# zgcr/SimpleAICV_pytorch_training_examples

Hardware: AMD Instinct MI355X
Metric: training images/sec/node (higher is better)
Workload: dtype bf16; 1 GPU; resnet50 3x224x224 synthetic training step (fwd+loss+bwd+all-reduce+optimizer), per-GPU batch 256; model=resnet50, global_batch=256, per_gpu_batch=256, parallelism=dp1, step_graph=True, bn_statistics=fixed-order partial rows, deterministic=True, loop=tools.scripts.train_classification, optimizer=SGD, param_groups=2

## Files before the change

### simpleaicv_pytorch_training_examples_amd/csrc/capi.hip

```cpp
#include <stdarg.h>
#include <stdio.h>
#include <string.h>

#include "common.h"
#include "saicv_internal.h"
#include "../../include/saicv_hip.h"

namespace saicv {

static thread_local char g_err[512] = "";

void set_error(const char* fmt, ...) {
    va_list ap;
    va_start(ap, fmt);
    vsnprintf(g_err, sizeof(g_err), fmt, ap);
    va_end(ap);
}

int check_launch(const char* what) {
    const hipError_t e = hipGetLastError();
    if (e != hipSuccess) {
        set_error("%s: launch failed: %s", what, hipGetErrorString(e));
        return -2;
    }
// ... 98 lines not shown
    return pack_weight(dtype, w, sO, sI, sR, sS, O, I, R, Sx, Ip, Op, wf, wd, S(stream));
}
int saicv_unpack_wgrad(const float* dw, int O, int I, int R, int Sx, int Ip, float* grad, long sO,
                       long sI, long sR, long sS, int accumulate, void* stream) {
    return unpack_wgrad(dw, O, I, R, Sx, Ip, grad, sO, sI, sR, sS, accumulate, S(stream));
}

int saicv_pack_weight_batched(int dtype, const saicv_pack_desc* descs, int n, int total_tiles, void* stream) {
    return pack_weight_batched(dtype, descs, n, total_tiles, S(stream));
}
int saicv_pack_input_s2d(int dtype, const float* src, long sN, long sC, long sH, long sW, void* dst, int N, int C, int H,
                         int W, int pad, int Cq, void* stream) {
    return pack_input_s2d(dtype, src, sN, sC, sH, sW, dst, N, C, H, W, pad, Cq, S(stream));
}
int saicv_pack_weight_s2d(int dtype, const float* w, long sO, long sI, long sR, long sS, int O, int I, int R, int Sx,
                          int Cq, void* wf, void* stream) {
    return pack_weight_s2d(dtype, w, sO, sI, sR, sS, O, I, R, Sx, Cq, wf, S(stream));
}
int saicv_unpack_wgrad_s2d(const float* dw, int O, int I, int R, int Sx, int Cq, float* grad, long sO, long sI, long sR,
                           long sS, int accumulate, void* stream) {
    return unpack_wgrad_s2d(dw, O, I, R, Sx, Cq, grad, sO, sI, sR, sS, accumulate, S(stream));
}

int saicv_conv2d_stat_rows(const saicv_conv_desc* d) {
    if (!d) return -1;
    return conv_stat_rows(d);
}

int saicv_conv2d_fwd(const saicv_conv_desc* d, const void* x, const void* wf, const float* bias,
                     void* y, int out_f32, float* stat_sum, float* stat_sq, void* stream) {
    if (check_desc(d, "saicv_conv2d_fwd")) return -1;
    SAICV_REQUIRE(!(stat_sum && out_f32), "saicv_conv2d_fwd: BN statistics need out_f32 = 0");
    const int M = d->N * d->OH * d->OW;
    return igemm_nt(d->dtype, 0, x, wf, y, bias, stat_sum, stat_sq, d->H, d->W, d->C, d->OH, d->OW,
                    d->R, d->S, d->stride, d->pad, M, d->K, d->R * d->S * d->C, d->K, out_f32, S(stream));
}

int saicv_conv2d_dgrad(const saicv_conv_desc* d, const void* dy, const void* wd, void* dx,
                       void* stream) {
    if (check_desc(d, "saicv_conv2d_dgrad")) return -1;
    const int M = d->N * d->H * d->W;
    return igemm_nt(d->dtype, 1, dy, wd, dx, nullptr, nullptr, nullptr, d->OH, d->OW, d->K, d->H, d->W,
                    d->R, d->S, d->stride, d->pad, M, d->C, d->R * d->S * d->K, d->C, 0, S(stream));
}

int saicv_conv2d_wgrad(const saicv_conv_desc* d, const void* dy, const void* x, float* dw,
                       void* stream) {
    if (check_desc(d, "saicv_conv2d_wgrad")) return -1;
    const int M = d->N * d->OH * d->OW;
    return igemm_tn(d->dtype, dy, x, dw, d->H, d->W, d->C, d->OH, d->OW, d->R, d->S, d->stride, d->pad,
                    M, d->K, d->R * d->S * d->C, S(stream));
}

int saicv_conv2d_wgrad_bias(const saicv_conv_desc* d, const void* dy, const void* x, float* dw, float* dbias,
                            void* stream) {
    if (check_desc(d, "saicv_conv2d_wgrad_bias")) return -1;
    const int M = d->N * d->OH * d->OW;
    return igemm_tn(d->dtype, dy, x, dw, d->H, d->W, d->C, d->OH, d->OW, d->R, d->S, d->stride, d->pad,
                    M, d->K, d->R * d->S * d->C, S(stream), dbias);
}

int saicv_linear_fwd(int dtype, const void* x, const void* wf, const float* bias, void* y, int M, int K, int N,
                     int out_f32, const void* addend, const float* row_scale, int rows_per_scale, void* stream) {
    EpiExtra ex;
    ex.addend = addend; ex.row_scale = row_scale; ex.rows_per_scale = rows_per_scale > 0 ? rows_per_scale : 1;
    return igemm_nt(dtype, 0, x, wf, y, bias, nullptr, nullptr, 1, 1, K, 1, 1, 1, 1, 1, 0, M, N, K, N, out_f32,
                    S(stream), (addend || row_scale) ? &ex : nullptr);
}
int saicv_linear_dgrad(int dtype, const void* dy, const void* wd, void* dx, int M, int K, int N, const void* addend,
                       void* stream) {
    EpiExtra ex;
    ex.addend = addend;
    return igemm_nt(dtype, 1, dy, wd, dx, nullptr, nullptr, nullptr, 1, 1, N, 1, 1, 1, 1, 1, 0, M, K, N, K, 0,
                    S(stream), addend ? &ex : nullptr);
}
int saicv_linear_gelu_fwd(int dtype, const void* x, const void* wf, const float* bias, void* y_pre, void* y_act, int M,
                          int K, int N, void* stream) {
    EpiExtra ex;
    ex.act_mode = 1; ex.out2 = y_act;
    return igemm_nt(dtype, 0, x, wf, y_pre, bias, nullptr, nullptr, 1, 1, K, 1, 1, 1, 1, 1, 0, M, N, K, N, 0, S(stream), &ex);
}
int saicv_linear_dgrad_gelu(int dtype, const void* dy, const void* wd, const void* pre, void* dx, int M, int K, int N,
                            void* stream) {
    EpiExtra ex;
    ex.act_mode = 2; ex.addend = pre;
    return igemm_nt(dtype, 1, dy, wd, dx, nullptr, nullptr, nullptr, 1, 1, N, 1, 1, 1, 1, 1, 0, M, K, N, K, 0, S(stream), &ex);
}
int saicv_linear_gelu_fwd_aux(int dtype, const void* x, const void* wf, const float* bias, void* y_dact, void* y_act, int M,
                              int K, int N, void* stream) {
    EpiExtra ex;
    ex.act_mode = 3; ex.out2 = y_act;
    return igemm_nt(dtype, 0, x, wf, y_dact, bias, nullptr, nullptr, 1, 1, K, 1, 1, 1, 1, 1, 0, M, N, K, N, 0, S(stream), &ex);
}
int saicv_linear_dgrad_mul(int dtype, const void* dy, const void* wd, const void* factor, void* dx, int M, int K, int N,
                           void* stream) {
    EpiExtra ex;
    ex.act_mode = 4; ex.addend = factor;
    return igemm_nt(dtype, 1, dy, wd, dx, nullptr, nullptr, nullptr, 1, 1, N, 1, 1, 1, 1, 1, 0, M, K, N, K, 0, S(stream), &ex);
}
int saicv_linear_wgrad(int dtype, const void* dy, const void* x, float* dw, float* dbias, int M, int K, int N,
                       void* stream) {
    return igemm_tn(dtype, dy, x, dw, 1, 1, K, 1, 1, 1, 1, 1, 0, M, N, K, S(stream), dbias);
}
int saicv_conv2d_dgrad_add(const saicv_conv_desc* d, const void* dy, const void* wd, const void* addend, void* dx,
                           void* stream) {
    if (check_desc(d, "saicv_conv2d_dgrad_add")) return -1;
// ... 312 lines not shown
```

### simpleaicv_pytorch_training_examples_amd/csrc/det.h

```cpp
#pragma once
#include <hip/hip_runtime.h>
#include <stddef.h>

namespace saicv {

extern int g_deterministic;

struct DetSink {
    float* part;
    size_t n;
};

__device__ __forceinline__ void det_add(const DetSink& s, float* dst_elem, size_t part_idx, int part_id, float v) {
    if (s.part) s.part[(size_t)part_id * s.n + part_idx] = v;
    else unsafeAtomicAdd(dst_elem, v);
}

struct DetParts {
    DetSink s{nullptr, 0};
    int nparts = 0;
    hipStream_t st = nullptr;
    int begin(hipStream_t stream, int parts, size_t n, const char* who, bool zero = true);
    int fold(float* dst, size_t offset, size_t count, bool wide = false) const;
    bool on() const { return s.part != nullptr; }
    const DetSink& sink() const { return s; }
};

}
```

### simpleaicv_pytorch_training_examples_amd/csrc/det.hip

```cpp
#include <mutex>

#include "common.h"
#include "det.h"

namespace saicv {

int g_deterministic = 0;

namespace {

struct StreamWs { hipStream_t st; float* p; size_t floats; };
constexpr size_t kInitialFloats = (size_t)24 << 20;
constexpr int MAX_STREAMS = 8;
StreamWs g_ws[MAX_STREAMS] = {};
int g_nws = 0;
StreamWs g_capture = {nullptr, nullptr, 0};
size_t g_max_floats = 0;
std::mutex g_mu;

bool is_capturing(hipStream_t st) {
    hipStreamCaptureStatus cap = hipStreamCaptureStatusNone;
    if (hipStreamIsCapturing(st, &cap) != hipSuccess) { (void)hipGetLastError(); return false; }
    return cap != hipStreamCaptureStatusNone;
}
// ... 48 lines not shown
    if (i >= count) return;
    const float* p = part + off + i;
    float acc = p[0];
    for (int k = 1; k < nparts; ++k) acc += p[(size_t)k * n];
    dst[i] += acc;
}
__global__ __launch_bounds__(256) void det_fold4_kernel(const float* __restrict__ part, size_t n, int nparts, size_t off, size_t count4,
                                                        float* __restrict__ dst) {
    const size_t i = (size_t)blockIdx.x * 256 + threadIdx.x;
    if (i >= count4) return;
    const float* p = part + off + i * 4;
    f32x4 acc = *reinterpret_cast<const f32x4*>(p);
    for (int k = 1; k < nparts; ++k) acc += *reinterpret_cast<const f32x4*>(p + (size_t)k * n);
    f32x4* d = reinterpret_cast<f32x4*>(dst + i * 4);
    *d = *d + acc;
}
constexpr int COOP_J = 8, COOP_E = 256 / COOP_J, COOP_CH = 32;
__global__ __launch_bounds__(256) void det_fold4_coop_kernel(const float* __restrict__ part, size_t n, int nparts, size_t off, size_t count4,
                                                             float* __restrict__ dst) {
    __shared__ f32x4 buf[2][COOP_CH][COOP_E];
    const int e = threadIdx.x % COOP_E, j = threadIdx.x / COOP_E;
    const size_t i = (size_t)blockIdx.x * COOP_E + e;
    const bool live = i < count4;
    const float* p = part + off + (live ? i : 0) * 4;
    const int chunks = (nparts + COOP_CH - 1) / COOP_CH;
    auto load = [&](int c) {
        f32x4 v[COOP_CH / COOP_J];
#pragma unroll
        for (int t = 0; t < COOP_CH / COOP_J; ++t) {
            const int k = c * COOP_CH + t * COOP_J + j;
            v[t] = (live && k < nparts) ? *reinterpret_cast<const f32x4*>(p + (size_t)k * n) : f32x4{0.f, 0.f, 0.f, 0.f};
        }
#pragma unroll
        for (int t = 0; t < COOP_CH / COOP_J; ++t) buf[c & 1][t * COOP_J + j][e] = v[t];
    };
    f32x4 acc = {0.f, 0.f, 0.f, 0.f};
    load(0);
    __syncthreads();
    for (int c = 0; c < chunks; ++c) {
        if (c + 1 < chunks) load(c + 1);
        if (j == 0) {
            const int cnt = min(COOP_CH, nparts - c * COOP_CH);
            int kk = 0;
            if (c == 0) { acc = buf[0][0][e]; kk = 1; }
            for (; kk < cnt; ++kk) acc += buf[c & 1][kk][e];
        }
        __syncthreads();
    }
    if (j == 0 && live) {
        f32x4* d = reinterpret_cast<f32x4*>(dst + i * 4);
        *d = *d + acc;
    }
}
constexpr int FOLD_J = 8, FOLD_E = 256 / FOLD_J;
__global__ __launch_bounds__(256) void det_fold4_wide_kernel(const float* __restrict__ part, size_t n, int nparts, size_t off, size_t count4,
                                                             float* __restrict__ dst) {
    __shared__ f32x4 red[FOLD_J][FOLD_E];
    const int e = threadIdx.x % FOLD_E, j = threadIdx.x / FOLD_E;
    const size_t i = (size_t)blockIdx.x * FOLD_E + e;
    f32x4 acc = {0.f, 0.f, 0.f, 0.f};
    if (i < count4) {
        const float* p = part + off + i * 4;
#pragma unroll 4
        for (int k = j; k < nparts; k += FOLD_J) acc += *reinterpret_cast<const f32x4*>(p + (size_t)k * n);
    }
    red[j][e] = acc;
    __syncthreads();
    if (j == 0 && i < count4) {
        f32x4 a = red[0][e];
#pragma unroll
        for (int jj = 1; jj < FOLD_J; ++jj) a += red[jj][e];
        f32x4* d = reinterpret_cast<f32x4*>(dst + i * 4);
        *d = *d + a;
    }
}

}

int DetParts::begin(hipStream_t stream, int parts, size_t n, const char* who, bool zero) {
    s = DetSink{nullptr, n};
    nparts = parts;
    st = stream;
    if (!g_deterministic || parts <= 1 || n == 0) return 0;
    float* p = ws_for(stream, (size_t)parts * n, who);
    if (!p) return -1;
    static const bool force = getenv("SAICV_ORDERED_ZERO") && atoi(getenv("SAICV_ORDERED_ZERO")) != 0;
    const bool clear = zero || force;
    if (clear && hipMemsetAsync(p, 0, (size_t)parts * n * sizeof(float), stream) != hipSuccess) {
        set_error("%s: clearing the deterministic workspace failed: %s", who, hipGetErrorString(hipGetLastError()));
        return -1;
    }
    s.part = p;
    return 0;
}

int DetParts::fold(float* dst, size_t offset, size_t count, bool wide_ok) const {
    if (!s.part || count == 0) return 0;
    const bool vec = (s.n % 4 == 0) && (offset % 4 == 0) && (count % 4 == 0) && ((uintptr_t)dst % 16 == 0);
    if (vec && wide_ok && nparts >= 4 * FOLD_J)
        hipLaunchKernelGGL(det_fold4_wide_kernel, dim3((unsigned)((count / 4 + FOLD_E - 1) / FOLD_E)), dim3(256), 0, st, s.part, s.n, nparts, offset, count / 4, dst);
    else if (vec && nparts >= COOP_CH)
        hipLaunchKernelGGL(det_fold4_coop_kernel, dim3((unsigned)((count / 4 + COOP_E - 1) / COOP_E)), dim3(256), 0, st, s.part, s.n, nparts, offset, count / 4, dst);
    else if (vec)
        hipLaunchKernelGGL(det_fold4_kernel, dim3((unsigned)((count / 4 + 255) / 256)), dim3(256), 0, st, s.part, s.n, nparts, offset, count / 4, dst);
    else
        hipLaunchKernelGGL(det_fold_kernel, dim3((unsigned)((count + 255) / 256)), dim3(256), 0, st, s.part, s.n, nparts, offset, count, dst);
    return check_launch("det_fold");
}

}

extern "C" {

int saicv_set_deterministic(int on) {
    const int prev = saicv::g_deterministic;
    saicv::g_deterministic = on ? 1 : 0;
    return prev;
}

int saicv_get_deterministic(void) { return saicv::g_deterministic; }

int saicv_deterministic_prepare(void* stream) {
    return saicv::ws_for((hipStream_t)stream, saicv::kInitialFloats, "deterministic_prepare") ? 0 : -1;
}

}
```

### simpleaicv_pytorch_training_examples_amd/csrc/igemm.hip

```cpp
#include <type_traits>

#include <stdlib.h>
#include "common.h"
#include "saicv_internal.h"
#include "det.h"
#include "../../include/saicv_hip.h"

namespace {

struct FastDiv {
    uint32_t mul, s1, s2;
};
DEVINL uint32_t fdiv(uint32_t n, FastDiv d) {
    const uint32_t t = __umulhi(d.mul, n);
    return (t + ((n - t) >> d.s1)) >> d.s2;
}

constexpr int nt_stages(int bm, int bn) { return (bm == 256 && bn == 128) ? 3 : 4; }
constexpr int nt_stages_kc8(int bm, int bn) { return (bm + bn) * 128 * 3 <= 150 * 1024 ? 3 : 2; }

struct NTParams {
    const void* src;
    const void* wgt;
    void* out;
// ... 753 lines not shown
        }
        __syncthreads();
        const size_t prow = (size_t)((MODE == 1 && cs > 1) ? blockIdx.y : 0) * p.bs_rows + tile_m;
        for (int c = tid; c < 2 * BN_T; c += NTHREADS) {
            const int which = c / BN_T, col = c - which * BN_T;
            float a = 0.f;
            for (int r = 0; r < RPP; ++r) a += red[(r * 2 + which) * BN_T + col];
            const int n = tile_n * BN_T + col;
            if (n < p.Nn) {
                float* dst = (which ? p.bs_gx : p.bs_g) + (p.stat_atomic_rows ? prow % p.stat_atomic_rows : prow) * (size_t)p.Nn + n;
                if (p.stat_atomic_rows) unsafeAtomicAdd(dst, a); else *dst = a;
            }
        }
    }
    }
#ifdef SAICV_NT_TIMELINE
    if (tl_on && tix == (int)blockIdx.x) {
        NT_STAMP(6);
        asm volatile("s_waitcnt vmcnt(0)" ::: "memory");
        NT_STAMP(7);
        if (tid == 0) {
            unsigned long long* rec = p.timeline + ((size_t)blockIdx.y * gridDim.x + blockIdx.x) * 16;
            unsigned int hw, xcc;
            asm volatile("s_getreg_b32 %0, hwreg(HW_REG_HW_ID)" : "=s"(hw));
            asm volatile("s_getreg_b32 %0, hwreg(HW_REG_XCC_ID)" : "=s"(xcc));
#pragma unroll
            for (int i = 0; i < 8; ++i) rec[i] = tl_t[i];
            rec[8] = ((unsigned long long)xcc << 32) | hw;
            rec[9] = __builtin_amdgcn_s_memrealtime();
            rec[10] = tl_rt0;
            rec[11] = tl_t[8]; rec[12] = tl_t[9]; rec[13] = tl_t[10];
        }
    }
#endif
    }
}


struct TNParams {
    const void* dy;
    const void* src;
    float* dw;
    float* dbias;
    uint32_t dy_bytes, src_bytes;
    int H, W, C;
    int OH, OW;
    int R, S, stride, pad;
    int M, Cout, Kd;
    int tiles_a, tiles_b;
    int m_per_split;
    int d_img, d_oh, d_ow;
    FastDiv fd_ohw, fd_ow;
    saicv::DetSink det;
};

template <typename T, int BA, int BB, int NWA, int NWB>
__global__ __launch_bounds__(64 * NWA * NWB) void igemm_tn_kernel(const TNParams p) {
    constexpr int THREADS = 64 * NWA * NWB;
    constexpr int EPC = ElemTraits<T>::EPC;
    constexpr int BR = 8 * EPC;
    constexpr int PITCH_A = (BA + 16) * (int)sizeof(T);
    constexpr int PITCH_B = (BB + 16) * (int)sizeof(T);
    constexpr int A_BYTES = BR * PITCH_A;
    constexpr int B_BYTES = BR * PITCH_B;
    constexpr int STAGE = A_BYTES + B_BYTES;
    constexpr int CPR_A = BA / EPC, CPR_B = BB / EPC;
    constexpr int RPP_A = THREADS / CPR_A, RPP_B = THREADS / CPR_B;
    constexpr int NA = BR / RPP_A, NB = BR / RPP_B;
    constexpr int WA = BA / NWA, WB = BB / NWB;
    constexpr int AT = WA / 16, BT = WB / 16;
    constexpr uint32_t OOB = 0xfffffff0u;

    extern __shared__ __attribute__((aligned(16))) char smem[];
    const int tid = threadIdx.x;
    const int lane = tid & 63;
    const int wave = tid >> 6;
    const int wa = wave % NWA, wb = wave / NWA;
    const int l15 = lane & 15, lg = lane >> 4;

    const int ntile = gridDim.x;
    const int lid = xcd_remap(blockIdx.y * ntile + blockIdx.x, ntile * gridDim.y);
    const int split = lid / ntile;
    const int tile = lid - split * ntile;
    const int tile_a = tile % p.tiles_a;
    const int tile_b = tile / p.tiles_a;
    const int m_begin = split * p.m_per_split;
    const int m_end = min(p.M, m_begin + p.m_per_split);
    if (m_begin >= m_end) return;

    const __amdgpu_buffer_rsrc_t dy_rs =
        __builtin_amdgcn_make_buffer_rsrc(const_cast<void*>(p.dy), 0, p.dy_bytes, 0x00020000);
    const __amdgpu_buffer_rsrc_t src_rs =
        __builtin_amdgcn_make_buffer_rsrc(const_cast<void*>(p.src), 0, p.src_bytes, 0x00020000);

    const int ca = tid % CPR_A, rba = tid / CPR_A;
    const int n_ld = tile_a * BA + ca * EPC;
    const bool n_ok = n_ld < p.Cout;
    uint32_t dy_off = (uint32_t)((m_begin + rba) * p.Cout + n_ld) * (uint32_t)sizeof(T);
    const uint32_t dy_row_step = (uint32_t)(RPP_A * p.Cout) * (uint32_t)sizeof(T);
    const uint32_t dy_tile_step = (uint32_t)(BR * p.Cout) * (uint32_t)sizeof(T);
    int m_a = m_begin + rba;
    const int cb = tid % CPR_B, rbb = tid / CPR_B;
    const int kk_ld = tile_b * BB + cb * EPC;
    const bool kk_ok = kk_ld < p.Kd;
    const int tap = kk_ld / p.C;
    const int c0 = kk_ld - tap * p.C;
    const int fr = tap / p.S - p.pad;
// ... 110 lines not shown
                    bf[bi] = u32x4{l2[0], l2[1], h2[0], h2[1]};
                }
#pragma unroll
                for (int ai = 0; ai < AT; ++ai)
#pragma unroll
                    for (int bi = 0; bi < BT; ++bi)
                        acc[ai][bi] = __builtin_amdgcn_mfma_f32_16x16x32_bf16(
                            __builtin_bit_cast(bf16x8, af[ai]), __builtin_bit_cast(bf16x8, bf[bi]),
                            acc[ai][bi], 0, 0, 0);
            }
        } else {
#pragma unroll
            for (int ks = 0; ks < BR / 4; ++ks) {
                float af[AT], bf[BT];
#pragma unroll
                for (int ai = 0; ai < AT; ++ai)
                    af[ai] = *reinterpret_cast<const float*>(base + fa_off[ai] + ks * 4 * PITCH_A);
#pragma unroll
                for (int bi = 0; bi < BT; ++bi)
                    bf[bi] = *reinterpret_cast<const float*>(base + fb_off[bi] + ks * 4 * PITCH_B);
#pragma unroll
                for (int ai = 0; ai < AT; ++ai)
#pragma unroll
                    for (int bi = 0; bi < BT; ++bi)
                        acc[ai][bi] = __builtin_amdgcn_mfma_f32_16x16x4f32(af[ai], bf[bi],
                                                                          acc[ai][bi], 0, 0, 0);
            }
        }
    };

    const int nt = (m_end - m_begin + BR - 1) / BR;
    load_tile();
    store_tile(0);
    __syncthreads();
    for (int t = 0; t < nt; ++t) {
        const int cur = t & 1;
        const bool more = (t + 1) < nt;
        if (more) load_tile();
        compute(cur);
        if (more) store_tile(cur ^ 1);
        __syncthreads();
    }

    if (do_bias) {
        float* red = reinterpret_cast<float*>(smem);
#pragma unroll
        for (int k = 0; k < EPC; ++k) red[tid * EPC + k] = bsum[k];
        __syncthreads();
        if (rba == 0 && n_ok) {
#pragma unroll
            for (int k = 0; k < EPC; ++k) {
                float sgm = 0.f;
                for (int t = 0; t < RPP_A; ++t) sgm += red[(t * CPR_A + ca) * EPC + k];
                saicv::det_add(p.det, p.dbias + n_ld + k, (size_t)p.Cout * p.Kd + n_ld + k, split, sgm);
            }
        }
    }
#pragma unroll
    for (int ai = 0; ai < AT; ++ai) {
        const int n0 = tile_a * BA + wa * WA + ai * 16 + lg * 4;
#pragma unroll
        for (int bi = 0; bi < BT; ++bi) {
            const int kk = tile_b * BB + wb * WB + bi * 16 + l15;
            if (kk < p.Kd) {
#pragma unroll
                for (int r = 0; r < 4; ++r)
                    if (n0 + r < p.Cout)
                        saicv::det_add(p.det, p.dw + (size_t)(n0 + r) * (size_t)p.Kd + kk, (size_t)(n0 + r) * (size_t)p.Kd + kk, split, acc[ai][bi][r]);
            }
        }
    }
}

DEVINL int tn_key(int r) { return (r & 3) | (((r >> 3) & 1) << 2); }
template <int CPR> DEVINL int tn_g(int r) { return CPR >= 16 ? tn_key(r) : (tn_key(r) >> 1); }

template <int BA, int BB, int NWA, int NWB, bool PLAIN>
__global__ __launch_bounds__(64 * NWA * NWB) void igemm_tn_dma_kernel(const TNParams p) {
    typedef bf16_t T;
    constexpr int NWAVES = NWA * NWB;
    constexpr int BR = 32;
    constexpr int CPR_A = BA / 8, CPR_B = BB / 8;
    constexpr int RPI_A = 64 / CPR_A, RPI_B = 64 / CPR_B;
    constexpr int NIA = (BR / RPI_A) / NWAVES, NIB = (BR / RPI_B) / NWAVES;
    static_assert(NIA >= 1 && NIB >= 1 && NIA * NWAVES * RPI_A == BR && NIB * NWAVES * RPI_B == BR, "tile / wavefront split");
    constexpr int LPT = NIA + NIB;
    constexpr int PITCH_A = BA * 2, PITCH_B = BB * 2;
    constexpr int A_BYTES = BR * PITCH_A, B_BYTES = BR * PITCH_B;
    constexpr int STAGE = A_BYTES + B_BYTES;
    constexpr int NSTAGE = 4;
    constexpr int WA = BA / NWA, WB = BB / NWB;
    constexpr int AT = WA / 16, BT = WB / 16;
    static_assert(AT % NWB == 0, "bias-gradient tiles per wavefront");
    constexpr int ABT = AT / NWB;
    constexpr uint32_t OOB = 0xfffffff0u;

    extern __shared__ __attribute__((aligned(16))) char smem[];
    const int tid = threadIdx.x;
    const int lane = tid & 63;
    const int wave = __builtin_amdgcn_readfirstlane(tid >> 6);
    const int wa = wave % NWA, wb = wave / NWA;
    const int l15 = lane & 15, lg = lane >> 4;

    const int ntile = gridDim.x;
    const int lid = xcd_remap(blockIdx.y * ntile + blockIdx.x, ntile * gridDim.y);
    const int split = lid / ntile;
    const int tile = lid - split * ntile;
    const int tile_a = tile % p.tiles_a;
    const int tile_b = tile / p.tiles_a;
    const int m_begin = split * p.m_per_split;
    const int m_end = min(p.M, m_begin + p.m_per_split);
    if (m_begin >= m_end) return;

    const __amdgpu_buffer_rsrc_t dy_rs =
        __builtin_amdgcn_make_buffer_rsrc(const_cast<void*>(p.dy), 0, p.dy_bytes, 0x00020000);
    const __amdgpu_buffer_rsrc_t src_rs =
        __builtin_amdgcn_make_buffer_rsrc(const_cast<void*>(p.src), 0, p.src_bytes, 0x00020000);

    uint32_t a_off[NIA];
    int a_m[NIA];
    bool a_ok[NIA];
#pragma unroll
    for (int i = 0; i < NIA; ++i) {
        const int row = (i * NWAVES + wave) * RPI_A + lane / CPR_A;
// ... 106 lines not shown
        for (int bi = 0; bi < BT; ++bi) {
            const uint32_t q = base + (uint32_t)fb_off[bi];
            asm volatile("ds_read_b64_tr_b16 %0, %2\n\tds_read_b64_tr_b16 %1, %2 offset:%3"
                         : "=&v"(blo[bi]), "=&v"(bhi[bi]) : "v"(q), "n"(4 * PITCH_B) : "memory");
        }
        u32x4 af[AT];
#pragma unroll
        for (int bi = 0; bi < BT; ++bi) {
            asm volatile("s_waitcnt lgkmcnt(%2)" : "+v"(blo[bi]), "+v"(bhi[bi]) : "n"(2 * (BT - 1 - bi)) : "memory");
            if (bi == 0) {
#pragma unroll
                for (int ai = 0; ai < AT; ++ai) af[ai] = u32x4{alo[ai][0], alo[ai][1], ahi[ai][0], ahi[ai][1]};
            }
            const u32x4 bf = {blo[bi][0], blo[bi][1], bhi[bi][0], bhi[bi][1]};
#pragma unroll
            for (int ai = 0; ai < AT; ++ai)
                acc[ai][bi] = __builtin_amdgcn_mfma_f32_16x16x32_bf16(__builtin_bit_cast(bf16x8, af[ai]),
                                                                      __builtin_bit_cast(bf16x8, bf), acc[ai][bi], 0, 0, 0);
        }
        if (do_bias) {
#pragma unroll
            for (int t = 0; t < ABT; ++t)
                bacc[t] = __builtin_amdgcn_mfma_f32_16x16x32_bf16(__builtin_bit_cast(bf16x8, af[wb * ABT + t]),
                                                                  __builtin_bit_cast(bf16x8, ones), bacc[t], 0, 0, 0);
        }
    };

    const int nt = (m_end - m_begin + BR - 1) / BR;
    int issued = 0;
    for (; issued < NSTAGE - 1 && issued < nt; ++issued) issue_step(issued);
    int st_c = 0;
    int st_i = issued % NSTAGE;
    for (int t = 0; t < nt; ++t) {
        const int ahead = issued - t - 1;
        if (ahead >= 2) asm volatile("s_waitcnt vmcnt(%0)" ::"n"(2 * LPT) : "memory");
        else if (ahead == 1) asm volatile("s_waitcnt vmcnt(%0)" ::"n"(LPT) : "memory");
        else asm volatile("s_waitcnt vmcnt(0)" ::: "memory");
        __builtin_amdgcn_s_barrier();
        if (issued < nt) {
            issue_step(st_i);
            ++issued;
            st_i = (st_i + 1 == NSTAGE) ? 0 : st_i + 1;
        }
        compute(st_c);
        st_c = (st_c + 1 == NSTAGE) ? 0 : st_c + 1;
    }

    if (do_bias && l15 == 0) {
#pragma unroll
        for (int t = 0; t < ABT; ++t) {
            const int n0 = tile_a * BA + wa * WA + (wb * ABT + t) * 16 + lg * 4;
#pragma unroll
            for (int r = 0; r < 4; ++r)
                if (n0 + r < p.Cout) saicv::det_add(p.det, p.dbias + n0 + r, (size_t)p.Cout * p.Kd + n0 + r, split, bacc[t][r]);
        }
    }
#pragma unroll
    for (int ai = 0; ai < AT; ++ai) {
        const int n0 = tile_a * BA + wa * WA + ai * 16 + lg * 4;
#pragma unroll
        for (int bi = 0; bi < BT; ++bi) {
            const int kk = tile_b * BB + wb * WB + bi * 16 + l15;
            if (kk < p.Kd) {
#pragma unroll
                for (int r = 0; r < 4; ++r)
                    if (n0 + r < p.Cout)
                        saicv::det_add(p.det, p.dw + (size_t)(n0 + r) * (size_t)p.Kd + kk, (size_t)(n0 + r) * (size_t)p.Kd + kk, split, acc[ai][bi][r]);
            }
        }
    }
}

FastDiv make_fastdiv(uint32_t d) {
    FastDiv f;
    uint32_t l = 0;
    while ((1ull << l) < d) ++l;
    f.mul = (uint32_t)(((1ull << 32) * ((1ull << l) - d)) / d + 1);
    f.s1 = l < 1 ? l : 1;
    f.s2 = l > 0 ? l - 1 : 0;
    return f;
}

template <typename K>
void allow_lds(K k, size_t smem) {
    hipFuncSetAttribute(reinterpret_cast<const void*>(k), hipFuncAttributeMaxDynamicSharedMemorySize, (int)smem);
}

template <typename T, int BM_T, int BN_T, int WM_, int WN_, int MODE, bool OUT_F32, bool PLAIN, int KC = 4>
int launch_nt1_inst(const NTParams& p, size_t smem, hipStream_t st) {
    auto k = igemm_nt1_kernel<T, BM_T, BN_T, WM_, WN_, MODE, OUT_F32, PLAIN, KC>;
    static bool once = (allow_lds(k, 160 * 1024), true);
    (void)once;
    dim3 grid(p.nblk, (MODE == 1 && p.stride > 1) ? p.stride * p.stride : 1), block(64 * WM_ * WN_);
    hipLaunchKernelGGL(k, grid, block, smem, st, p);
    return saicv::check_launch("igemm_nt");
}

template <typename T, int BM_T, int BN_T, int WM_, int WN_, int MODE>
int launch_nt1(const NTParams& p, bool out_f32, bool plain, hipStream_t st) {
    constexpr bool F32_OUT = !(BM_T == 256 && BN_T == 256) && (sizeof(T) == 4 || MODE == 0);
    constexpr bool BF16_OUT = sizeof(T) == 2;
    constexpr size_t smem_full = nt_stages(BM_T, BN_T) * (size_t)(BM_T * 64 + BN_T * 64);
    const size_t epi = BM_T * (size_t)(BN_T * ((out_f32 || sizeof(T) == 4) ? 4 : 2) + 16) +
                       2 * WM_ * BN_T * sizeof(float);
    size_t smem = smem_full;
    if (smem < epi) smem = epi;
#ifdef SAICV_NT_TIMELINE
    if (getenv("SAICV_NT_SOLO") && smem < 84 * 1024) smem = 84 * 1024;
#endif
    if constexpr (BF16_OUT && BM_T == 256) {
        if (p.kc8 && plain && !out_f32) {
            constexpr size_t ring = nt_stages_kc8(BM_T, BN_T) * (size_t)(BM_T + BN_T) * 128;
            return launch_nt1_inst<T, BM_T, BN_T, WM_, WN_, MODE, false, true, 8>(p, ring < epi ? epi : ring, st);
        }
    }
    if constexpr (F32_OUT) {
        if (out_f32) {
            if (plain) return launch_nt1_inst<T, BM_T, BN_T, WM_, WN_, MODE, true, true>(p, smem, st);
            return launch_nt1_inst<T, BM_T, BN_T, WM_, WN_, MODE, true, false>(p, smem, st);
        }
    }
    if constexpr (BF16_OUT) {
        if (!out_f32) {
// ... 59 lines not shown
    if (streamable && q.R == 1 && q.S == 1 && q.pad == 0) {
        pl.blocks = saicv::pw_stream_blocks(q.dtype, q.M, q.Nn, q.Kd, (q.addend || q.bn_sums) && !q.stats);
        if (pl.blocks > 0) {
            pl.route = NT_PW_STREAM;
            pl.stat_rows = pl.blocks;
            return pl;
        }
    }
    if (streamable && q.R == 3 && q.S == 3 && q.pad == 1 && q.C == 64 && q.H == q.OH && q.W == q.OW && q.H >= 1 && q.W >= 1 &&
        q.M % (q.H * q.W) == 0) {
        pl.blocks = saicv::pw3_stream_blocks(q.dtype, q.M, q.Nn, q.Kd);
        if (pl.blocks > 0) {
            pl.route = NT_PW3_STREAM;
            pl.stat_rows = pl.blocks;
            return pl;
        }
    }
    const bool f32o = q.out_f32 || q.dtype == SAICV_DTYPE_F32;
    int M_tile = q.M;
    if (q.mode == 1 && q.stride > 1)
        M_tile = (q.M / (q.OH * q.OW)) * ((q.OH + q.stride - 1) / q.stride) * ((q.OW + q.stride - 1) / q.stride);
    const int bk = q.dtype == SAICV_DTYPE_BF16 ? 32 : 16;
    pl.tile = pick_tile(M_tile, q.Nn, (q.Kd + bk - 1) / bk, f32o);
    const char* ke = getenv("SAICV_NT_KC8");
    const int kc8_mode = ke ? atoi(ke) : 2;
    const bool pointwise = q.R == 1 && q.S == 1 && q.pad == 0 && (q.mode == 0 || q.stride == 1);
    pl.plain = pointwise;
    pl.f32o = f32o;
    const bool ok = q.dtype == SAICV_DTYPE_BF16 && !f32o && pointwise && kTiles[pl.tile].bm == 256 && q.Kd >= 256;
    if (ok && kc8_mode == 1) pl.kc8 = true;
    const bool rule_ok = (kc8_mode == 2 && q.act_mode == 0) || kc8_mode == 3;
    if (ok && rule_ok && q.Nn >= 2048 && q.Nn % 256 == 0 && q.Kd >= 512 && (long)((M_tile + 255) / 256) * (q.Nn / 256) >= 4 * 256) {
        pl.kc8 = true;
        pl.tile = 0;
    }
    const int classes = q.mode == 1 && q.stride > 1 ? q.stride * q.stride : 1;
    pl.stat_rows = ((M_tile + kTiles[pl.tile].bm - 1) / kTiles[pl.tile].bm) * classes;
    pl.blocks = pl.stat_rows * ((q.Nn + kTiles[pl.tile].bn - 1) / kTiles[pl.tile].bn);
    return pl;
}

bool nt_operands_fit(const NTProblem& q) {
    const size_t esz = q.dtype == SAICV_DTYPE_BF16 ? 2 : 4;
    const size_t src_bytes = (size_t)(q.M / (q.OH * q.OW)) * q.H * q.W * q.C * esz;
    const size_t wgt_bytes = (size_t)q.Nn * q.Kd * esz;
    return src_bytes < 0xfffffff0ull && wgt_bytes < 0xfffffff0ull;
}

struct TNProblem {
    int dtype;
    int H, W, C, OH, OW, R, S, stride, pad;
    int M, Cout, Kd;
};
struct TNPlan {
    bool big;
    int ba, bb;
    int tiles_a, tiles_b;
    int BR;
    int total_rt;
    int rt_per;
    int splits;
    bool dma;
    bool plain;
};

TNPlan tn_plan(const TNProblem& q) {
    TNPlan pl;
    const int epc = q.dtype == SAICV_DTYPE_BF16 ? 8 : 4;
    const int M = q.M, Cout = q.Cout, Kd = q.Kd;
    const int BR = 8 * epc;
    pl.BR = BR;
    const int big_tiles = ((Cout + 255) / 256) * ((Kd + 255) / 256);
    const int big_steps = ((M + BR - 1) / BR) / (256 / big_tiles > 0 ? 256 / big_tiles : 1);
    const bool big = Cout % 256 == 0 && Kd >= 256 && (Kd % 256 == 0 || Kd >= 1024) && big_steps >= 48;
    pl.big = big;
    const int ba = big ? 256 : Cout <= 64 ? 64 : 128;
    const int bb = big ? 256 : Kd <= 64 ? 64 : 128;
    pl.ba = ba; pl.bb = bb;
    pl.tiles_a = (Cout + ba - 1) / ba;
    pl.tiles_b = (Kd + bb - 1) / bb;
    const int tiles = pl.tiles_a * pl.tiles_b;
    const int total_rt = (M + BR - 1) / BR;
    const char* slots_env = getenv("SAICV_TN_SLOTS_PCT");
    const int slots_pct = slots_env ? atoi(slots_env) : (g_saicv_comm_world > 1 ? 85 : 100);
    int splits = ((big ? 256 : 512) * slots_pct / 100) / tiles;
    if (splits > total_rt) splits = total_rt;
    if (splits < 1) splits = 1;
    int rt_per = (total_rt + splits - 1) / splits;
    splits = (total_rt + rt_per - 1) / rt_per;
    pl.total_rt = total_rt; pl.rt_per = rt_per; pl.splits = splits;
    const char* de = getenv("SAICV_TN_DMA");
    const int use_dma = de ? atoi(de) : 1;
    pl.dma = use_dma && q.dtype == SAICV_DTYPE_BF16;
    pl.plain = q.R == 1 && q.S == 1 && q.stride == 1 && q.pad == 0 && q.H == q.OH && q.W == q.OW;
    return pl;
}

bool tn_operands_fit(const TNProblem& q) {
    const size_t esz = q.dtype == SAICV_DTYPE_BF16 ? 2 : 4;
    const size_t dy_bytes = (size_t)q.M * q.Cout * esz;
    const size_t src_bytes = (size_t)(q.M / (q.OH * q.OW)) * q.H * q.W * q.C * esz;
    return dy_bytes < 0xfffffff0ull && src_bytes < 0xfffffff0ull;
}

template <typename T, int BA, int BB, int NWA = 2, int NWB = 2>
int launch_tn(const TNParams& p, int splits, hipStream_t st) {
    constexpr int EPC = ElemTraits<T>::EPC;
    constexpr int BR = 8 * EPC;
    constexpr size_t smem = 2 * (size_t)BR * ((BA + 16) + (BB + 16)) * sizeof(T);
    dim3 grid(p.tiles_a * p.tiles_b, splits), block(64 * NWA * NWB);
    auto k = igemm_tn_kernel<T, BA, BB, NWA, NWB>;
    static bool once = (allow_lds(k, smem), true);
    (void)once;
    hipLaunchKernelGGL(k, grid, block, smem, st, p);
    return saicv::check_launch("igemm_tn");
}

template <int BA, int BB, int NWA = 2, int NWB = 2>
int launch_tn_dma(const TNParams& p, int splits, bool plain, hipStream_t st) {
    constexpr size_t smem = 4 * (size_t)32 * (BA + BB) * 2;
    dim3 grid(p.tiles_a * p.tiles_b, splits), block(64 * NWA * NWB);
    if (plain) {
        auto k = igemm_tn_dma_kernel<BA, BB, NWA, NWB, true>;
        static bool once = (allow_lds(k, smem), true);
        (void)once;
        hipLaunchKernelGGL(k, grid, block, smem, st, p);
    } else {
// ... 70 lines not shown
        SAICV_REQUIRE(p.act_mode >= 1 && p.act_mode <= 4, "igemm_nt: act_mode %d", p.act_mode);
        SAICV_REQUIRE((p.act_mode & 1) ? p.out2 != nullptr : p.addend != nullptr, "igemm_nt: fused GELU operand missing");
        SAICV_REQUIRE(stat_sum == nullptr && p.row_scale == nullptr, "igemm_nt: fused GELU excludes BN statistics / row scale");
    }
    if (p.addend || p.row_scale) {
        const int osz = (out_f32 || dtype == SAICV_DTYPE_F32) ? 4 : 2;
        SAICV_REQUIRE((ldo * osz) % 16 == 0, "igemm_nt: fused residual needs a 16-byte aligned leading dimension");
        SAICV_REQUIRE(p.rows_per_scale >= 1, "igemm_nt: rows_per_scale must be >= 1");
    }
    const NTProblem q = {dtype, mode, H, W, C, OH, OW, R, S, stride, pad, M, Nn, Kd, ldo, out_f32 != 0,
                         bias != nullptr, stat_sum != nullptr, p.addend != nullptr, p.row_scale != nullptr, p.out2 != nullptr,
                         p.bs_y != nullptr, p.act_mode};
    const NTPlan pl = nt_plan(q);
    const bool f32o = out_f32 != 0 || dtype == SAICV_DTYPE_F32;
    static const long min_mb = getenv("SAICV_NT_STREAM_MIN_MB") ? atol(getenv("SAICV_NT_STREAM_MIN_MB")) : 0;
    const int stream_out = (size_t)M * Nn * (f32o ? 4 : 2) >= (size_t)min_mb * 1024 * 1024 ? 1 : 0;
    if (pl.route == NT_PW_STREAM)
        return pw_stream(M, Nn, Kd, src, wgt, out, stat_sum, stat_sq, p.stat_atomic_rows, ex, stream_out, pl.blocks, st);
    if (pl.route == NT_PW3_STREAM)
        return pw3_stream(mode, M, H, W, src, wgt, out, stat_sum, stat_sq, p.stat_atomic_rows, ex, stream_out, pl.blocks, st);
    p.H = H; p.W = W; p.C = C; p.OH = OH; p.OW = OW; p.R = R; p.S = S; p.stride = stride; p.pad = pad;
    p.M = M; p.Nn = Nn; p.Kd = Kd; p.ldo = ldo;
    const size_t esz = dtype == SAICV_DTYPE_BF16 ? 2 : 4;
    SAICV_REQUIRE(nt_operands_fit(q), "igemm_nt: operand larger than 4 GiB (buffer addressing)");
    p.src_bytes = (uint32_t)((size_t)(M / (OH * OW)) * H * W * C * esz);
    p.wgt_bytes = (uint32_t)((size_t)Nn * Kd * esz);
    p.fd_ohw = make_fastdiv((uint32_t)(OH * OW));
    p.fd_ow = make_fastdiv((uint32_t)OW);
    p.stream_out = stream_out;
    p.kc8 = pl.kc8 ? 1 : 0;
    const NTTile& g = kTiles[pl.tile];
    const int classes = mode == 1 && stride > 1 ? stride * stride : 1;
    p.bs_rows = pl.stat_rows / classes;
    p.tiles_n = (Nn + g.bn - 1) / g.bn;
    p.nblk = p.tiles_n * p.bs_rows;
#define NT_DISPATCH(TT, MODE_)                                                              \
    switch (pl.tile) {                                                                      \
        case 0: return launch_nt1<TT, 256, 256, 2, 4, MODE_>(p, f32o, pl.plain, st);                  \
        case 1: return launch_nt1<TT, 256, 128, 4, 2, MODE_>(p, f32o, pl.plain, st);                  \
        case 2: return launch_nt1<TT, 128, 128, 2, 2, MODE_>(p, f32o, pl.plain, st);                  \
        default: return launch_nt1<TT, 128, 64, 2, 2, MODE_>(p, f32o, pl.plain, st);                  \
    }
    if (dtype == SAICV_DTYPE_BF16) {
        if (mode == 0) { NT_DISPATCH(bf16_t, 0) } else { NT_DISPATCH(bf16_t, 1) }
    } else {
        if (mode == 0) { NT_DISPATCH(float, 0) } else { NT_DISPATCH(float, 1) }
    }
#undef NT_DISPATCH
}

static int igemm_tn_launch(int dtype, TNParams& p, const TNPlan& pl, hipStream_t st);

int igemm_tn(int dtype, const void* dy, const void* src, float* dw, int H, int W, int C, int OH,
             int OW, int R, int S, int stride, int pad, int M, int Cout, int Kd, hipStream_t st, float* dbias) {
    const int epc = dtype == SAICV_DTYPE_BF16 ? 8 : 4;
    SAICV_REQUIRE(C % epc == 0 && Cout % epc == 0, "igemm_tn: C=%d, Cout=%d must be multiples of %d", C, Cout, epc);
    SAICV_REQUIRE(M > 0 && Cout > 0 && Kd > 0, "igemm_tn: empty problem");
    TNParams p;
    p.dy = dy; p.src = src; p.dw = dw; p.dbias = dbias; p.H = H; p.W = W; p.C = C; p.OH = OH; p.OW = OW;
    p.R = R; p.S = S; p.stride = stride; p.pad = pad; p.M = M; p.Cout = Cout; p.Kd = Kd;
    const TNProblem q = {dtype, H, W, C, OH, OW, R, S, stride, pad, M, Cout, Kd};
    const size_t esz = dtype == SAICV_DTYPE_BF16 ? 2 : 4;
    SAICV_REQUIRE(tn_operands_fit(q), "igemm_tn: operand larger than 4 GiB (buffer addressing)");
    p.dy_bytes = (uint32_t)((size_t)M * Cout * esz);
    p.src_bytes = (uint32_t)((size_t)(M / (OH * OW)) * H * W * C * esz);
    p.fd_ohw = make_fastdiv((uint32_t)(OH * OW));
    p.fd_ow = make_fastdiv((uint32_t)OW);
    const TNPlan pl = tn_plan(q);
    p.tiles_a = pl.tiles_a;
    p.tiles_b = pl.tiles_b;
    p.m_per_split = pl.rt_per * pl.BR;
    DetParts det;
    if (det.begin(st, pl.splits, (size_t)Cout * Kd + (dbias ? Cout : 0), "igemm_tn", false)) return -1;
    p.det = det.sink();
    const int rc = igemm_tn_launch(dtype, p, pl, st);
    if (rc) return rc;
    if (det.fold(dw, 0, (size_t)Cout * Kd, true)) return -1;
    if (dbias && det.fold(dbias, (size_t)Cout * Kd, (size_t)Cout)) return -1;
    return 0;
}

static int igemm_tn_launch(int dtype, TNParams& p, const TNPlan& pl, hipStream_t st) {
    const int OW = p.OW;
    const int ohw = p.OH * OW;
    const int splits = pl.splits, ba = pl.ba, bb = pl.bb;
    const bool big = pl.big;
    p.d_img = pl.BR / ohw;
    const int rem = pl.BR - p.d_img * ohw;
    p.d_oh = rem / OW;
    p.d_ow = rem - p.d_oh * OW;
    if (pl.dma) {
        const int br = 32;
        p.d_img = br / ohw;
        const int rem32 = br - p.d_img * ohw;
        p.d_oh = rem32 / OW;
        p.d_ow = rem32 - p.d_oh * OW;
        const bool plain = pl.plain;
        if (big) return launch_tn_dma<256, 256, 2, 4>(p, splits, plain, st);
        if (ba == 64 && bb == 64) return launch_tn_dma<64, 64>(p, splits, plain, st);
        if (ba == 64) return launch_tn_dma<64, 128>(p, splits, plain, st);
        if (bb == 64) return launch_tn_dma<128, 64>(p, splits, plain, st);
        return launch_tn_dma<128, 128>(p, splits, plain, st);
    }
    if (big) {
        if (dtype == SAICV_DTYPE_BF16) return launch_tn<bf16_t, 256, 256, 2, 4>(p, splits, st);
        return launch_tn<float, 256, 256, 2, 4>(p, splits, st);
    }
    if (dtype == SAICV_DTYPE_BF16) {
        if (ba == 64 && bb == 64) return launch_tn<bf16_t, 64, 64>(p, splits, st);
        if (ba == 64) return launch_tn<bf16_t, 64, 128>(p, splits, st);
        if (bb == 64) return launch_tn<bf16_t, 128, 64>(p, splits, st);
        return launch_tn<bf16_t, 128, 128>(p, splits, st);
    } else {
        if (ba == 64 && bb == 64) return launch_tn<float, 64, 64>(p, splits, st);
        if (ba == 64) return launch_tn<float, 64, 128>(p, splits, st);
        if (bb == 64) return launch_tn<float, 128, 64>(p, splits, st);
        return launch_tn<float, 128, 128>(p, splits, st);
    }
}

static NTProblem nt_problem_of(const saicv_plan_query* q) {
    const saicv_conv_desc* d = &q->conv;
    const bool out2 = q->act_mode == 1 || q->act_mode == 3;
    switch (q->op) {
        case SAICV_PLAN_CONV_FWD:
            return {d->dtype, 0, d->H, d->W, d->C, d->OH, d->OW, d->R, d->S, d->stride, d->pad, d->N * d->OH * d->OW, d->K,
                    d->R * d->S * d->C, d->K, q->out_f32 != 0, q->bias != 0, q->stats != 0, q->addend != 0, q->row_scale != 0, out2,
                    q->bn_sums != 0, q->act_mode};
        case SAICV_PLAN_CONV_DGRAD:
            return {d->dtype, 1, d->OH, d->OW, d->K, d->H, d->W, d->R, d->S, d->stride, d->pad, d->N * d->H * d->W, d->C,
                    d->R * d->S * d->K, d->C, false, false, false, q->addend != 0, false, false, q->bn_sums != 0, 0};
// ... 56 lines not shown
```

### simpleaicv_pytorch_training_examples_amd/csrc/saicv_internal.h

```cpp
#pragma once
#include <hip/hip_runtime.h>

struct saicv_conv_desc;
struct saicv_plan_query;
struct saicv_plan;

namespace saicv {

void set_error(const char* fmt, ...);
int check_launch(const char* what);

int conv_stat_rows(const saicv_conv_desc* d);
struct EpiExtra {
    const void* addend = nullptr;
    const float* row_scale = nullptr;
    int rows_per_scale = 1;
    int act_mode = 0;
    void* out2 = nullptr;
    const uint8_t* addend_gate = nullptr;
    const void* bs_y = nullptr;
    const uint8_t* bs_mask = nullptr;
    const float* bs_mean = nullptr;
    const float* bs_invstd = nullptr;
    float* bs_g = nullptr;
    float* bs_gx = nullptr;
    int stat_atomic_rows = 0;
};
int conv_bwd_stat_rows(const saicv_conv_desc* d);
int igemm_nt(int dtype, int mode, const void* src, const void* wgt, void* out, const float* bias,
             float* stat_sum, float* stat_sq, int H, int W, int C, int OH, int OW, int R, int S,
             int stride, int pad, int M, int Nn, int Kd, int ldo, int out_f32, hipStream_t st,
             const EpiExtra* ex = nullptr);
int igemm_tn(int dtype, const void* dy, const void* src, float* dw, int H, int W, int C, int OH,
             int OW, int R, int S, int stride, int pad, int M, int Cout, int Kd, hipStream_t st,
             float* dbias = nullptr);

int igemm_plan(const saicv_plan_query* q, saicv_plan* out);

int pw_stream_blocks(int dtype, int M, int Nn, int Kd, bool fused_dgrad);
int pw_stream(int M, int Nn, int Kd, const void* src, const void* wgt, void* out, float* stat_sum, float* stat_sq,
              int stat_atomic_rows, const EpiExtra* ex, int stream_out, int blocks, hipStream_t st);
int pw3_stream_blocks(int dtype, int M, int Nn, int Kd);
int pw3_stream(int mode, int M, int H, int W, const void* src, const void* wgt, void* out, float* stat_sum, float* stat_sq,
               int stat_atomic_rows, const EpiExtra* ex, int stream_out, int blocks, hipStream_t st);

int window_partition(int dtype, const void* x, void* out, int B, int H, int W, int C, int ws, hipStream_t st);
int window_unpartition(int dtype, const void* win, const void* addend, void* out, int B, int H, int W, int C, int ws,
                       hipStream_t st);
int relpos_fwd(int dtype, const void* q, long q_rs, long q_bs, const float* tab_h, const float* tab_w, float* rel_h,
               float* rel_w, int B, int heads, int Sh, int Sw, hipStream_t st);
int relpos_bwd(int dtype, const void* q, void* dq, long q_rs, long q_bs, const float* tab_h, const float* tab_w,
               const float* d_rel_h, const float* d_rel_w, float* dtab_h, float* dtab_w, float* ws, int B, int heads, int Sh,
               int Sw, hipStream_t st);
size_t relpos_bwd_ws_floats(int Sh, int Sw);
int mask_loss_stats(int dtype, const void* logits, const float* targets, float* stats, int B, int M, size_t HW,
                    double alpha, double gamma, double thr, hipStream_t st);
int mask_loss_grad(int dtype, const void* logits, const float* targets, const float* coef, void* dlogits, int B, int M,
                   size_t HW, double alpha, double gamma, hipStream_t st);
int hyper_product_fwd(int dtype, const void* x, const void* hyper, void* out, int B, int Tm, int P, int C, hipStream_t st);
int hyper_product_bwd(int dtype, const void* x, const void* hyper, const void* dout, void* dx, float* dhyper, int B, int Tm,
                      int P, int C, hipStream_t st);
int upsample4_fwd(int dtype, const void* low, void* out, int planes, int h, int w, hipStream_t st);
int upsample4_bwd(int dtype, const void* dhi, void* dlow, int planes, int h, int w, hipStream_t st);
int mask_loss_stats_up4(int dtype, const void* low, const float* targets, float* stats, int B, int M, int h, int w,
                        double alpha, double gamma, double thr, hipStream_t st);
int mask_loss_grad_up4(int dtype, const void* low, const float* targets, const float* coef, void* dlow, int B, int M, int h,
                       int w, double alpha, double gamma, hipStream_t st);
int attention_stream(int dtype, int D, int which, const void* desc, hipStream_t st);

}
```

Baseline: 12630 images/s.

## Write wgrad split partials in packed MFMA tile layout and fold with a scatter kernel

In deterministic mode the weight-gradient GEMM now stores each split's partial accumulators as contiguous f32x4 per lane in a tile-packed layout instead of scattered scalar stores into a row-major Cout x Kd buffer. A new fold kernel reads the packed partials with vector loads, reduces across splits (using a wide cooperative variant when there are many splits), and scatters the sums into dw. The plan also lowers the threshold for choosing the big 256x256 tile in deterministic mode, which gives fewer splits and less partial traffic. A debug entry point for forcing the big or small tile choice is added.

```diff
diff --git a/simpleaicv_pytorch_training_examples_amd/csrc/capi.hip b/simpleaicv_pytorch_training_examples_amd/csrc/capi.hip
--- a/simpleaicv_pytorch_training_examples_amd/csrc/capi.hip
+++ b/simpleaicv_pytorch_training_examples_amd/csrc/capi.hip
@@ -174,6 +174,13 @@
                     M, d->K, d->R * d->S * d->C, S(stream));
 }
 
+int saicv_debug_conv2d_wgrad_form(const saicv_conv_desc* d, const void* dy, const void* x, float* dw, void* stream, int big) {
+    if (check_desc(d, "saicv_debug_conv2d_wgrad_form")) return -1;
+    const int M = d->N * d->OH * d->OW;
+    return igemm_tn(d->dtype, dy, x, dw, d->H, d->W, d->C, d->OH, d->OW, d->R, d->S, d->stride, d->pad,
+                    M, d->K, d->R * d->S * d->C, S(stream), nullptr, big != 0);
+}
+
 int saicv_conv2d_wgrad_bias(const saicv_conv_desc* d, const void* dy, const void* x, float* dw, float* dbias,
                             void* stream) {
     if (check_desc(d, "saicv_conv2d_wgrad_bias")) return -1;
diff --git a/simpleaicv_pytorch_training_examples_amd/csrc/det.h b/simpleaicv_pytorch_training_examples_amd/csrc/det.h
--- a/simpleaicv_pytorch_training_examples_amd/csrc/det.h
+++ b/simpleaicv_pytorch_training_examples_amd/csrc/det.h
@@ -16,12 +16,15 @@
     else unsafeAtomicAdd(dst_elem, v);
 }
 
+constexpr int FOLD_TN_WIDE_FROM = 8;
+__host__ __device__ inline size_t tn_packed_floats(int Cout, int Kd) { return (size_t)((Cout + 15) / 16) * ((Kd + 15) / 16) * 256; }
 struct DetParts {
     DetSink s{nullptr, 0};
     int nparts = 0;
     hipStream_t st = nullptr;
     int begin(hipStream_t stream, int parts, size_t n, const char* who, bool zero = true);
-    int fold(float* dst, size_t offset, size_t count, bool wide = false) const;
+    int fold(float* dst, size_t offset, size_t count) const;
+    int fold_tn(float* dw, int Cout, int Kd) const;
     bool on() const { return s.part != nullptr; }
     const DetSink& sink() const { return s; }
 };
diff --git a/simpleaicv_pytorch_training_examples_amd/csrc/det.hip b/simpleaicv_pytorch_training_examples_amd/csrc/det.hip
--- a/simpleaicv_pytorch_training_examples_amd/csrc/det.hip
+++ b/simpleaicv_pytorch_training_examples_amd/csrc/det.hip
@@ -124,26 +124,42 @@
         *d = *d + acc;
     }
 }
-constexpr int FOLD_J = 8, FOLD_E = 256 / FOLD_J;
-__global__ __launch_bounds__(256) void det_fold4_wide_kernel(const float* __restrict__ part, size_t n, int nparts, size_t off, size_t count4,
-                                                             float* __restrict__ dst) {
-    __shared__ f32x4 red[FOLD_J][FOLD_E];
-    const int e = threadIdx.x % FOLD_E, j = threadIdx.x / FOLD_E;
-    const size_t i = (size_t)blockIdx.x * FOLD_E + e;
+template <int J>
+__global__ __launch_bounds__(256) void det_fold_tn_kernel(const float* __restrict__ part, size_t n, int nparts, size_t quads, int Cout,
+                                                          int Kd, float* __restrict__ dw) {
+    constexpr int E = 256 / J;
+    __shared__ f32x4 red[J][E];
+    const int e = threadIdx.x % E, j = threadIdx.x / E;
+    const size_t i = (size_t)blockIdx.x * E + e;
+    const int kb16 = (Kd + 15) / 16;
+    const int lane = (int)(i % 64);
+    const size_t blk = i / 64;
+    const int n0 = (int)(blk / kb16) * 16 + (lane >> 4) * 4, kk = (int)(blk % kb16) * 16 + (lane & 15);
+    const bool live = i < quads && n0 < Cout && kk < Kd;
     f32x4 acc = {0.f, 0.f, 0.f, 0.f};
-    if (i < count4) {
-        const float* p = part + off + i * 4;
+    if (live) {
+        const float* p = part + i * 4;
+        if (J == 1) {
+            acc = *reinterpret_cast<const f32x4*>(p);
+            for (int k = 1; k < nparts; ++k) acc += *reinterpret_cast<const f32x4*>(p + (size_t)k * n);
+        } else {
 #pragma unroll 4
-        for (int k = j; k < nparts; k += FOLD_J) acc += *reinterpret_cast<const f32x4*>(p + (size_t)k * n);
-    }
-    red[j][e] = acc;
-    __syncthreads();
-    if (j == 0 && i < count4) {
-        f32x4 a = red[0][e];
-#pragma unroll
-        for (int jj = 1; jj < FOLD_J; ++jj) a += red[jj][e];
-        f32x4* d = reinterpret_cast<f32x4*>(dst + i * 4);
-        *d = *d + a;
+            for (int k = j; k < nparts; k += J) acc += *reinterpret_cast<const f32x4*>(p + (size_t)k * n);
+        }
+    }
+    if (J > 1) {
+        red[j][e] = acc;
+        __syncthreads();
+        if (j == 0 && live) {
+            acc = red[0][e];
+#pragma unroll
+            for (int jj = 1; jj < J; ++jj) acc += red[jj][e];
+        }
+    }
+    if (j == 0 && live) {
+        float* d = dw + (size_t)n0 * Kd + kk;
+#pragma unroll
+        for (int r = 0; r < 4; ++r) d[(size_t)r * Kd] += acc[r];
     }
 }
 
@@ -166,12 +182,10 @@
     return 0;
 }
 
-int DetParts::fold(float* dst, size_t offset, size_t count, bool wide_ok) const {
+int DetParts::fold(float* dst, size_t offset, size_t count) const {
     if (!s.part || count == 0) return 0;
     const bool vec = (s.n % 4 == 0) && (offset % 4 == 0) && (count % 4 == 0) && ((uintptr_t)dst % 16 == 0);
-    if (vec && wide_ok && nparts >= 4 * FOLD_J)
-        hipLaunchKernelGGL(det_fold4_wide_kernel, dim3((unsigned)((count / 4 + FOLD_E - 1) / FOLD_E)), dim3(256), 0, st, s.part, s.n, nparts, offset, count / 4, dst);
-    else if (vec && nparts >= COOP_CH)
+    if (vec && nparts >= COOP_CH)
         hipLaunchKernelGGL(det_fold4_coop_kernel, dim3((unsigned)((count / 4 + COOP_E - 1) / COOP_E)), dim3(256), 0, st, s.part, s.n, nparts, offset, count / 4, dst);
     else if (vec)
         hipLaunchKernelGGL(det_fold4_kernel, dim3((unsigned)((count / 4 + 255) / 256)), dim3(256), 0, st, s.part, s.n, nparts, offset, count / 4, dst);
@@ -180,6 +194,16 @@
     return check_launch("det_fold");
 }
 
+int DetParts::fold_tn(float* dw, int Cout, int Kd) const {
+    if (!s.part) return 0;
+    const size_t quads = tn_packed_floats(Cout, Kd) / 4;
+    if (nparts >= FOLD_TN_WIDE_FROM)
+        hipLaunchKernelGGL(det_fold_tn_kernel<8>, dim3((unsigned)((quads + 31) / 32)), dim3(256), 0, st, s.part, s.n, nparts, quads, Cout, Kd, dw);
+    else
+        hipLaunchKernelGGL(det_fold_tn_kernel<1>, dim3((unsigned)((quads + 255) / 256)), dim3(256), 0, st, s.part, s.n, nparts, quads, Cout, Kd, dw);
+    return check_launch("det_fold_tn");
+}
+
 }
 
 extern "C" {
diff --git a/simpleaicv_pytorch_training_examples_amd/csrc/igemm.hip b/simpleaicv_pytorch_training_examples_amd/csrc/igemm.hip
--- a/simpleaicv_pytorch_training_examples_amd/csrc/igemm.hip
+++ b/simpleaicv_pytorch_training_examples_amd/csrc/igemm.hip
@@ -829,7 +829,40 @@
     int d_img, d_oh, d_ow;
     FastDiv fd_ohw, fd_ow;
     saicv::DetSink det;
+    size_t bias_off;
 };
+
+template <int AT, int BT>
+DEVINL void tn_epilogue(const TNParams& p, int split, int n_wave, int kk_wave, int lane, const f32x4 (&acc)[AT][BT]) {
+    const int l15 = lane & 15, lg = lane >> 4;
+    if (p.det.part) {
+        const int nb16 = (p.Cout + 15) >> 4, kb16 = (p.Kd + 15) >> 4;
+        float* part = p.det.part + (size_t)split * p.det.n + lane * 4;
+#pragma unroll
+        for (int ai = 0; ai < AT; ++ai) {
+            const int nb = (n_wave >> 4) + ai;
+#pragma unroll
+            for (int bi = 0; bi < BT; ++bi) {
+                const int kb = (kk_wave >> 4) + bi;
+                if (nb < nb16 && kb < kb16) *reinterpret_cast<f32x4*>(part + ((size_t)nb * kb16 + kb) * 256) = acc[ai][bi];
+            }
+        }
+        return;
+    }
+#pragma unroll
+    for (int ai = 0; ai < AT; ++ai) {
+        const int n0 = n_wave + ai * 16 + lg * 4;
+#pragma unroll
+        for (int bi = 0; bi < BT; ++bi) {
+            const int kk = kk_wave + bi * 16 + l15;
+            if (kk < p.Kd) {
+#pragma unroll
+                for (int r = 0; r < 4; ++r)
+                    if (n0 + r < p.Cout) unsafeAtomicAdd(p.dw + (size_t)(n0 + r) * (size_t)p.Kd + kk, acc[ai][bi][r]);
+            }
+        }
+    }
+}
 
 template <typename T, int BA, int BB, int NWA, int NWB>
 __global__ __launch_bounds__(64 * NWA * NWB) void igemm_tn_kernel(const TNParams p) {
@@ -1046,24 +1079,11 @@
             for (int k = 0; k < EPC; ++k) {
                 float sgm = 0.f;
                 for (int t = 0; t < RPP_A; ++t) sgm += red[(t * CPR_A + ca) * EPC + k];
-                saicv::det_add(p.det, p.dbias + n_ld + k, (size_t)p.Cout * p.Kd + n_ld + k, split, sgm);
-            }
-        }
-    }
-#pragma unroll
-    for (int ai = 0; ai < AT; ++ai) {
-        const int n0 = tile_a * BA + wa * WA + ai * 16 + lg * 4;
-#pragma unroll
-        for (int bi = 0; bi < BT; ++bi) {
-            const int kk = tile_b * BB + wb * WB + bi * 16 + l15;
-            if (kk < p.Kd) {
-#pragma unroll
-                for (int r = 0; r < 4; ++r)
-                    if (n0 + r < p.Cout)
-                        saicv::det_add(p.det, p.dw + (size_t)(n0 + r) * (size_t)p.Kd + kk, (size_t)(n0 + r) * (size_t)p.Kd + kk, split, acc[ai][bi][r]);
-            }
-        }
-    }
+                saicv::det_add(p.det, p.dbias + n_ld + k, p.bias_off + n_ld + k, split, sgm);
+            }
+        }
+    }
+    tn_epilogue<AT, BT>(p, split, tile_a * BA + wa * WA, tile_b * BB + wb * WB, lane, acc);
 }
 
 DEVINL int tn_key(int r) { return (r & 3) | (((r >> 3) & 1) << 2); }
@@ -1276,23 +1296,10 @@
             const int n0 = tile_a * BA + wa * WA + (wb * ABT + t) * 16 + lg * 4;
 #pragma unroll
             for (int r = 0; r < 4; ++r)
-                if (n0 + r < p.Cout) saicv::det_add(p.det, p.dbias + n0 + r, (size_t)p.Cout * p.Kd + n0 + r, split, bacc[t][r]);
-        }
-    }
-#pragma unroll
-    for (int ai = 0; ai < AT; ++ai) {
-        const int n0 = tile_a * BA + wa * WA + ai * 16 + lg * 4;
-#pragma unroll
-        for (int bi = 0; bi < BT; ++bi) {
-            const int kk = tile_b * BB + wb * WB + bi * 16 + l15;
-            if (kk < p.Kd) {
-#pragma unroll
-                for (int r = 0; r < 4; ++r)
-                    if (n0 + r < p.Cout)
-                        saicv::det_add(p.det, p.dw + (size_t)(n0 + r) * (size_t)p.Kd + kk, (size_t)(n0 + r) * (size_t)p.Kd + kk, split, acc[ai][bi][r]);
-            }
-        }
-    }
+                if (n0 + r < p.Cout) saicv::det_add(p.det, p.dbias + n0 + r, p.bias_off + n0 + r, split, bacc[t][r]);
+        }
+    }
+    tn_epilogue<AT, BT>(p, split, tile_a * BA + wa * WA, tile_b * BB + wb * WB, lane, acc);
 }
 
 FastDiv make_fastdiv(uint32_t d) {
@@ -1458,6 +1465,7 @@
     int H, W, C, OH, OW, R, S, stride, pad;
     int M, Cout, Kd;
 };
+constexpr int TN_DET_BIG_STEPS = 8;
 struct TNPlan {
     bool big;
     int ba, bb;
@@ -1470,7 +1478,7 @@
     bool plain;
 };
 
-TNPlan tn_plan(const TNProblem& q) {
+TNPlan tn_plan(const TNProblem& q, int debug_big = -1) {
     TNPlan pl;
     const int epc = q.dtype == SAICV_DTYPE_BF16 ? 8 : 4;
     const int M = q.M, Cout = q.Cout, Kd = q.Kd;
@@ -1478,7 +1486,9 @@
     pl.BR = BR;
     const int big_tiles = ((Cout + 255) / 256) * ((Kd + 255) / 256);
     const int big_steps = ((M + BR - 1) / BR) / (256 / big_tiles > 0 ? 256 / big_tiles : 1);
-    const bool big = Cout % 256 == 0 && Kd >= 256 && (Kd % 256 == 0 || Kd >= 1024) && big_steps >= 48;
+    const bool fits = Cout % 256 == 0 && Kd >= 256 && (Kd % 256 == 0 || Kd >= 1024);
+    bool big = fits && big_steps >= (saicv::g_deterministic ? TN_DET_BIG_STEPS : 48);
+    if (debug_big >= 0) big = fits && debug_big != 0;
     pl.big = big;
     const int ba = big ? 256 : Cout <= 64 ? 64 : 128;
     const int bb = big ? 256 : Kd <= 64 ? 64 : 128;
@@ -1655,7 +1665,7 @@
 static int igemm_tn_launch(int dtype, TNParams& p, const TNPlan& pl, hipStream_t st);
 
 int igemm_tn(int dtype, const void* dy, const void* src, float* dw, int H, int W, int C, int OH,
-             int OW, int R, int S, int stride, int pad, int M, int Cout, int Kd, hipStream_t st, float* dbias) {
+             int OW, int R, int S, int stride, int pad, int M, int Cout, int Kd, hipStream_t st, float* dbias, int debug_big) {
     const int epc = dtype == SAICV_DTYPE_BF16 ? 8 : 4;
     SAICV_REQUIRE(C % epc == 0 && Cout % epc == 0, "igemm_tn: C=%d, Cout=%d must be multiples of %d", C, Cout, epc);
     SAICV_REQUIRE(M > 0 && Cout > 0 && Kd > 0, "igemm_tn: empty problem");
@@ -1669,17 +1679,18 @@
     p.src_bytes = (uint32_t)((size_t)(M / (OH * OW)) * H * W * C * esz);
     p.fd_ohw = make_fastdiv((uint32_t)(OH * OW));
     p.fd_ow = make_fastdiv((uint32_t)OW);
-    const TNPlan pl = tn_plan(q);
+    const TNPlan pl = tn_plan(q, debug_big);
     p.tiles_a = pl.tiles_a;
     p.tiles_b = pl.tiles_b;
     p.m_per_split = pl.rt_per * pl.BR;
     DetParts det;
-    if (det.begin(st, pl.splits, (size_t)Cout * Kd + (dbias ? Cout : 0), "igemm_tn", false)) return -1;
+    p.bias_off = saicv::tn_packed_floats(Cout, Kd);
+    if (det.begin(st, pl.splits, p.bias_off + (dbias ? Cout : 0), "igemm_tn", false)) return -1;
     p.det = det.sink();
     const int rc = igemm_tn_launch(dtype, p, pl, st);
     if (rc) return rc;
-    if (det.fold(dw, 0, (size_t)Cout * Kd, true)) return -1;
-    if (dbias && det.fold(dbias, (size_t)Cout * Kd, (size_t)Cout)) return -1;
+    if (det.fold_tn(dw, Cout, Kd)) return -1;
+    if (dbias && det.fold(dbias, p.bias_off, (size_t)Cout)) return -1;
     return 0;
 }
 
diff --git a/simpleaicv_pytorch_training_examples_amd/csrc/saicv_internal.h b/simpleaicv_pytorch_training_examples_amd/csrc/saicv_internal.h
--- a/simpleaicv_pytorch_training_examples_amd/csrc/saicv_internal.h
+++ b/simpleaicv_pytorch_training_examples_amd/csrc/saicv_internal.h
@@ -33,7 +33,7 @@
              const EpiExtra* ex = nullptr);
 int igemm_tn(int dtype, const void* dy, const void* src, float* dw, int H, int W, int C, int OH,
              int OW, int R, int S, int stride, int pad, int M, int Cout, int Kd, hipStream_t st,
-             float* dbias = nullptr);
+             float* dbias = nullptr, int debug_big = -1);
 
 int igemm_plan(const saicv_plan_query* q, saicv_plan* out);
 
```

Measured after the change: 12690 images/s (median of 6 runs). Within noise of the previous version (+0.5%).
